# datemoon/ASR-decoder

Hardware: AMD Instinct MI355X
Metric: frames/sec decoded (RTFx = value/100) at fixed beam (higher is better)
Workload: dtype f32; 1 GPU; BASELINE configs[1]: batch=128 utterances/GPU x 300 frames, 10142717-arc HCLG, beam=13, max_active=1000000, min_active=0, 3000 pdfs; global_batch=128, frames_per_utt=300, parallelism=utterance-sharded x1 (graph replicated), channel_groups=3, degraded_frames=0, regime=beam-only pruning (max_active never binds, min_active 0): bi

## Files before the change

### asr-decoder_amd/csrc/wfst_kernels.hip

```cpp
#include <type_traits>

#include "wfst_device.h"

namespace wfst {

typedef unsigned long long u64;

__device__ __forceinline__ uint32_t f2o(float f) {
  uint32_t u = __float_as_uint(f);
  return u ^ ((u >> 31) ? 0xFFFFFFFFu : 0x80000000u);
}
__device__ __forceinline__ float o2f(uint32_t o) {
  uint32_t u = (o & 0x80000000u) ? (o ^ 0x80000000u) : ~o;
  return __uint_as_float(u);
}
template <class T>
__device__ __forceinline__ T ld_agent(const T *p) {
  return __hip_atomic_load(p, __ATOMIC_RELAXED, __HIP_MEMORY_SCOPE_AGENT);
}
__device__ __forceinline__ void lds_barrier() {
  asm volatile("s_waitcnt lgkmcnt(0)" ::: "memory");
  __builtin_amdgcn_s_barrier();
  asm volatile("" ::: "memory");
}
// ... 831 lines not shown
            const bool pseudo = pi >= 0;
            const int a = abeg_[q] + off;
            const int4 arc = arc_[q];
            const float base_cost = (cost_[q] + (-ll_[q])) + __int_as_float(arc.z);
            int4 rec;
            if (pseudo) {
              const int4 leaf = (j + 1 < S) ? s_arc[j + 1] : D.g.arcs[a + 1];
              float tt = base_cost;
              if (leaf.z == 1) {
                tt = tt + __int_as_float(leaf.y);
              } else if (leaf.z == 2) {
                tt = (tt + __int_as_float(leaf.w)) + __int_as_float(leaf.y);
              } else {
                const float *pw = D.g.pseudo_w + (size_t)arc.y * kPseudoDepthMax;
                for (int u = 0; u < leaf.z; ++u) tt = tt + pw[u];
              }
              rec = make_int4(arc.w, __float_as_int(tt), kPrevUnresolved, (int)((uint32_t)leaf.x | kEpsRec));
            } else {
              rec = make_int4(arc.w, __float_as_int(base_cost), tok0 + (super ? s_tidx[l] : l), (int)((uint32_t)a | flags_of((uint32_t)arc.y)));
              tmin = fminf(tmin, base_cost);
            }
            if (D.degcode) {
              const uint32_t code = (uint32_t)arc.x >> kColBits;
              rec.w = (int)(((uint32_t)rec.w & 0x3FFFFFFFu) | (code << 30));
              rec.z = pseudo ? kPrevUnresolved - (int)(code >> 2) : (int)((uint32_t)rec.z | ((code >> 2) << D.tok_idx_bits));
            }
            s_arc[j] = rec;
            cand_mask |= 1u << i;
            if (D.best_exp) {
              const u64 cb = ((u64)f2o(__int_as_float(rec.y)) << 32) | (uint32_t)rec.x;
              cbest = cb < cbest ? cb : cbest;
            }
          }
        }
        {
          const float wmin = wave_min_f(tmin);
          if (lane == 0 && wmin < kInf) atomicMin(&s_bound, f2o(wmin + ab));
          if (D.best_exp) {
            const u64 cv = cbest < best_seen ? cbest : ~0ull;
            if (__ballot(cv != ~0ull)) {
              const u64 wb = wave_min_u64(cv);
              if (lane == 0) atomicMin(&s_best, wb);
            }
          }
          lds_barrier();
          const uint32_t tb = s_bound;
          if (o2f(tb) < bound) {
            if (tid == 0) atomicMin(&ctl->bound, tb);
            bound = o2f(tb);
          }
          if (D.best_exp && tid == 0) {
            const u64 tbest = s_best;
            if (tbest < best_seen) atomicMin(&ctl->best_next, tbest);
          }
        }
        if constexpr (kTimers) { if (tid == 0) dbg_phase(D, 14, tq); }
        ST_FRESH_TID();
        int pr[kStIter];
#pragma unroll
        for (int i = 0; i < kStIter; ++i) {
          pr[i] = -1;
          if (!(cand_mask & (1u << i))) continue;
          const int j = (wave + i * (kStThreads / 64)) * 64 + lane;
          const int2 xy = *reinterpret_cast<const int2 *>(&s_arc[j]);
          if (__int_as_float(xy.y) < bound) {
            const int part = part_of(hash32(xy.x), log2part);
            pr[i] = (part << 16) | atomicAdd(&s_cnt[part], 1);
          }
        }
        lds_barrier();
        if (tid < 64) {
          const int cnt = tid < P ? s_cnt[tid] : 0;
          int g = 0;
          if (cnt) {
            g = atomicAdd(&bucket_cnt[tid], cnt);
            if (g + cnt > bcap) atomicOr(&ctl->error, kErrBucketFull);
          }
          s_gbase[tid] = g;
          s_cnt[tid] = 0;
          const uint32_t wrote = wave_sum_u32((uint32_t)cnt);
          if (tid == 0 && wrote) atomicAdd(&s_stat[2], wrote);
        }
        lds_barrier();
        if constexpr (kTimers) { if (tid == 0) dbg_phase(D, 15, tq); }
        ST_FRESH_TID();
#pragma unroll
        for (int i = 0; i < kStIter; ++i) {
          if (pr[i] < 0) continue;
          const int j = (wave + i * (kStThreads / 64)) * 64 + lane;
          const int p = pr[i] >> 16, gi = s_gbase[p] + (pr[i] & 0xFFFF);
          if (gi < bcap) bucket[(size_t)p * bcap + gi] = s_arc[j];
        }
        __syncthreads();
        if (tid == 0) { s_bound = 0xFFFFFFFFu; s_best = ~0ull; }
        if constexpr (kTimers) { if (tid == 0) dbg_phase(D, 16, tq); }
      }
      if ((rnd + 1) * kStTokens < n_live) {
        const bool exp = s_cost[tid] <= cutoff;
        const int nem = s_nemit[tid], zt = (s_base[tid + 1] - s_base[tid] - nem) >> 1;
        const uint32_t wN = (uint32_t)__popcll(__ballot(exp)), wE = wave_sum_u32(exp ? (uint32_t)nem : 0u),
                       wZ = wave_sum_u32(exp ? (uint32_t)zt : 0u);
        if (lane == 0) { if (wN) atomicAdd(&s_stat[0], wN); if (wE) atomicAdd(&s_stat[1], wE); if (wZ) atomicAdd(&s_stat[3], wZ); }
        __syncthreads();
      }
      }
    }
    {
      ST_FRESH_TID();
      const bool exp = counted && s_cost[tid] <= cutoff;
      const int nem = exp ? s_nemit[tid] : 0, zt = exp ? (s_base[tid + 1] - s_base[tid] - nem) >> 1 : 0;
      tile_tail(D, c, ctl, group, par, exp ? 1u : 0u, (uint32_t)nem, 0u, (uint32_t)zt, s_stat);
    }
    if (total_tiles <= (int)gridDim.x) break;
    if (tid == 0) s_ticket = (int)gridDim.x + atomicAdd(&fc->ticket[par], 1);
    __syncthreads();
    t = __builtin_amdgcn_readfirstlane(s_ticket);
    __syncthreads();
    if (t < total_tiles) td = tiles[t];
    if constexpr (kTimers) tq = wall_clock64();
  }
}
#undef ST_FRESH_TID
__global__ __launch_bounds__(kStThreads, 4) void expand_kernel_staged(DecoderDev D, int group, int par) { expand_staged_body<false, false>(D, group, par); }
__global__ __launch_bounds__(kStThreads, 4) void expand_kernel_staged_timed(DecoderDev D, int group, int par) { expand_staged_body<true, false>(D, group, par); }
#pragma clang diagnostic push
#pragma clang diagnostic ignored "-Wpass-failed"
__global__ __launch_bounds__(kStThreads, 5) void expand_kernel_staged_row(DecoderDev D, int group, int par) { expand_staged_body<false, true>(D, group, par); }
#pragma clang diagnostic pop
__global__ __launch_bounds__(kStThreads, 4) void expand_kernel_staged_row_timed(DecoderDev D, int group, int par) { expand_staged_body<true, true>(D, group, par); }

constexpr int kInsertThreads = 512;
#ifndef WFST_INSERT_UNROLL
#define WFST_INSERT_UNROLL 3
#endif
constexpr int kInsertUnroll = WFST_INSERT_UNROLL;
constexpr uint32_t kNoSlot = 0xFFFFu;
constexpr int kInsertPk = (kInsertUnroll + 1) / 2;
__device__ __forceinline__ void put16(uint32_t *p, int k, uint32_t v) {
  p[k >> 1] = (k & 1) ? (p[k >> 1] & 0xFFFFu) | (v << 16) : (p[k >> 1] & 0xFFFF0000u) | v;
}
__device__ __forceinline__ uint32_t get16(const uint32_t *p, int k) { return (k & 1) ? p[k >> 1] >> 16 : p[k >> 1] & 0xFFFFu; }

struct BoundaryLite {
  float redf[16];
  u64 best;
  int active, n, nd, front_begin, ntiles, tile_tokens, tile_start, pad_bits;
  uint32_t hist[256];
  uint32_t sel_prefix, sel_k;
  float prev_ab;
  u64 h_best;
  int h_risky;
  int h_nf, h_err;
  uint32_t h_bound;
};
template <int kT>
__device__ __forceinline__ void frame_boundary_fused(const DecoderDev &D, int c, const int32_t *target, int chan_cnt, int group,
                                                     int par_next, bool do_prep, BoundaryLite &sh, uint32_t *sel_cache, int sel_cache_cap);
template <int kT, bool kSc1, class Sh, int kKeep>
__device__ __forceinline__ float kth_smallest_t(const int4 *tok, int n, int k, Sh &sh, uint32_t *cache, int cache_cap, uint32_t lo_o, uint32_t hi_o);
#ifndef WFST_NOINLINE_COLD
#define WFST_COLD __forceinline__
#else
#define WFST_COLD __attribute__((noinline))
#endif
#ifndef WFST_COLD_KEEP
#define WFST_COLD_KEEP 4
#endif
template <int kT>
__device__ WFST_COLD float kth_smallest_cold(const int4 *tok, int n, int k, BoundaryLite *sh, uint32_t *cache, int cache_cap, uint32_t lo_o, uint32_t hi_o) {
  return kth_smallest_t<kT, true, BoundaryLite, WFST_COLD_KEEP>(tok, n, k, *sh, cache, cache_cap, lo_o, hi_o);
}

template <bool kLat, bool kBig, bool kFused>
__device__ __forceinline__ void insert_body(const DecoderDev &D, int group, int par, const int32_t *target = nullptr, int boundary = 0,
                                            int chan_cnt = 0) {
  constexpr bool kTwo = kFused && !kLat && !kBig;
  extern __shared__ __attribute__((aligned(16))) unsigned char smem[];
  const int tid = threadIdx.x, lane = tid & 63, wave = tid >> 6;
  const int SLmax = D.lds_slots;
  typedef typename std::conditional<kBig, u64, int32_t>::type KeyT;
  const KeyT kNoKey = (KeyT)~(KeyT)0;
  u64 *vals = reinterpret_cast<u64 *>(smem);
  KeyT *keys = reinterpret_cast<KeyT *>(smem + (size_t)SLmax * 8);
  int32_t *tidx = reinterpret_cast<int32_t *>(smem + (size_t)SLmax * (8 + sizeof(KeyT)));
  struct __attribute__((aligned(16))) InsertShared {
    int nstates, gpos, wpos, ok, item, pad[3];
    int lw[12];
    u64 best[kInsertThreads / 64];
    int pref[68];
  };
  static_assert(sizeof(InsertShared) % 16 == 0, "keep the dynamic LDS base aligned");
  __shared__ InsertShared ish;
  int &s_nstates = ish.nstates, &s_gpos = ish.gpos, &s_wpos = ish.wpos, &s_ok = ish.ok, &s_item = ish.item, &s_last = ish.pad[0];
  int &s_ech = ish.pad[1], &s_efill = ish.pad[2];
  constexpr bool kListEmit = kLat && kFused && !kBig;
  __shared__ BoundaryLite bsh;
  u64 *s_best = ish.best;
  int *s_pref = ish.pref;
  FrameCtl *fc = D.fctl + group;
  const int n_heavy = min(fc->n_items[par], D.item_cap / 2), n_items = n_heavy + min(fc->n_small[par], D.item_cap / 2);
  const int P = D.n_part;

  unsigned long long th = wall_clock64();
  for (int it = blockIdx.x; it < n_items;) {
  const int islot = __builtin_amdgcn_readfirstlane(it < n_heavy ? it : D.item_cap - 1 - (it - n_heavy));
  const int item = D.items[(size_t)group * D.item_cap + islot];
  const int my_pref = D.item_pref[((size_t)group * D.item_cap + islot) * 64 + lane];
  const int c = item >> 16, g0 = (item >> 8) & 0xFF, G = item & 0xFF;
  ChanCtl *ctl = D.ctl + c;
  int ech_reg = 0;
  if (kListEmit && tid == 0) {
    s_efill = 0;
    if (G) ech_reg = atomicAdd(&D.emit_cnt[c * 32], kEmitChunk);
  }
  int n = 0;
  {
    n = G ? __shfl(my_pref, G - 1, 64) : 0;
    if (wave == 0 && lane < G) s_pref[lane + 1] = my_pref;
    if (tid == 0) s_pref[0] = 0;
  }
  int log2g = 0;
  while ((1 << log2g) < G) ++log2g;
  const int log2grp = D.log2part - log2g;
  const int4 *bucket0 = D.bucket + ((size_t)c * P + g0) * D.bucket_cap;
  const int32_t *bucket_lm0 = kBig ? D.bucket_lm + ((size_t)c * P + g0) * D.bucket_cap : nullptr;
  const uint32_t bound_o = ctl->bound;
  const float cutoff = o2f(bound_o);
  const u64 best_early = (kTwo && D.best_exp) ? ctl->best_next : ~0ull;
  const int err_early = kTwo ? ctl->error : 0;
  const bool risky = kTwo && boundary && (ctl->items_left & kRiskyBit);
  int log2sl = 6;
  while ((1 << log2sl) < 4 * n && log2sl < D.log2lds) ++log2sl;
  const int SL = 1 << log2sl;
  const uint32_t mask = (uint32_t)SL - 1;
  const int base = ctl->front_begin + ctl->front_count;
  int4 *tok = D.tok + (size_t)c * D.arena_cap;
  u64 *evals = D.eps_vals + (size_t)c * D.ecap;
  int32_t *etoki = D.eps_toki + (size_t)c * D.ecap;
  int32_t *eocc = D.eps_occ_list + (size_t)c * D.wl_cap;
  int4 *wl = D.worklist + (size_t)c * 2 * D.wl_cap;
  u64 *occ_wl = reinterpret_cast<u64 *>(&ctl->eps_occ);

  int log2sub = 0;
  while (n > ((SL * 3) >> 2) << log2sub) ++log2sub;
  const int sub_shift = 32 - log2grp - log2sl - log2sub;
  if (sub_shift < 0 && tid == 0) atomicOr(&ctl->error, kErrTableFull);
  __syncthreads();
  auto load_rec = [&](int i, int *lm) -> int4 {
    *lm = 0;
    if (i >= n) return make_int4(0, 0x7F800000, 0, 0);
    int b = 0;
    if (G > 1) {
      int lo = 0, hi = G;
      while (hi - lo > 1) {
        const int mid = (lo + hi) >> 1;
        if (s_pref[mid] <= i) lo = mid; else hi = mid;
      }
      b = lo;
    }
    const size_t pos = (size_t)b * D.bucket_cap + (i - s_pref[b]);
    if constexpr (kBig) *lm = bucket_lm0[pos];
    return bucket0[pos];
  };
  auto key_of = [&](const int4 &r, int lm) -> KeyT {
    if constexpr (kBig) return big_key(r.x, lm);
    else return (KeyT)r.x;
  };
  auto hash_of = [&](const int4 &r, int lm) -> uint32_t { return kBig ? hash_big(r.x, lm) : hash32(r.x); };

  u64 best = ~0ull;
  if (tid == 0) dbg_phase(D, 22, th);
  unsigned long long tq = wall_clock64();
  for (int sub = 0; sub_shift >= 0 && sub < (1 << log2sub); ++sub) {
    __syncthreads();
    int4 r[kInsertUnroll];
    int rl[kInsertUnroll];
#pragma unroll
    for (int k = 0; k < kInsertUnroll; ++k) r[k] = load_rec(k * kInsertThreads + tid, &rl[k]);
    for (int i = tid; i < SL; i += kInsertThreads) { keys[i] = kNoKey; vals[i] = kEmptyVal; }
    if (tid == 0) { s_nstates = 0; s_wpos = 0; s_ok = 1; }
    __syncthreads();
    if (tid == 0) dbg_phase(D, 6, tq);
#ifndef WFST_RECORDS_AT_FIRST_USE
    if constexpr (kTwo) {
#pragma unroll
      for (int k = 0; k < kInsertUnroll; ++k) asm volatile("" ::"v"(r[k].x), "v"(r[k].y), "v"(r[k].z), "v"(r[k].w));
    }
#endif

    const bool one_sweep = n <= kInsertThreads * kInsertUnroll;
    const bool carry = one_sweep && SL <= 0x8000;
    uint32_t cs[kInsertPk];
#pragma unroll
    for (int j = 0; j < kInsertPk; ++j) cs[j] = ~0u;
    for (int i0 = 0; i0 < n; i0 += kInsertThreads * kInsertUnroll) {
      if (i0 > 0) {
#pragma unroll
        for (int k = 0; k < kInsertUnroll; ++k) r[k] = load_rec(i0 + k * kInsertThreads + tid, &rl[k]);
      }
#pragma unroll
      for (int k = 0; k < kInsertUnroll; ++k) {
        if (!(__int_as_float(r[k].y) < cutoff)) continue;
        const uint32_t h = hash_of(r[k], rl[k]);
        if (log2sub && (int)((h >> sub_shift) & ((1u << log2sub) - 1u)) != sub) continue;
        uint32_t slot = lds_slot_of(h, log2grp, log2sl);
        const KeyT key = key_of(r[k], rl[k]);
        bool found = false;
        for (int q = 0; q < SL; ++q) {
          KeyT kk = keys[slot];
          if (kk == kNoKey) {
            kk = atomicCAS(&keys[slot], kNoKey, key);
            if (kk == kNoKey) { atomicAdd(&s_nstates, 1); found = true; break; }
          }
          if (kk == key) { found = true; break; }
          slot = (slot + 1) & mask;
        }
        if (found) {
          atomicMin(&vals[slot], ((u64)f2o(__int_as_float(r[k].y)) << 32) | (uint32_t)r[k].w);
          put16(cs, k, slot & 0xFFFFu);
        } else atomicOr(&ctl->error, kErrTableFull);
      }
    }
    __syncthreads();
    if (tid == 0) dbg_phase(D, 7, tq);
    const int ns = s_nstates;
    if (tid == 0) {
      int g = atomicAdd(&ctl->new_count, ns);
      s_gpos = g;
      if constexpr (kListEmit) s_ech = ech_reg;
      if (!(kTwo && D.soft_limit) && g + ns > D.max_tok) { atomicOr(&ctl->error, kErrFrontierFull); s_ok = 0; }
      if ((int64_t)base + g + ns > D.arena_cap) { atomicOr(&ctl->error, kErrArenaFull); s_ok = 0; }
      if (kTwo && !s_ok) atomicOr(reinterpret_cast<u64 *>(&ctl->new_count), kFrameErrBit);
    }
    __syncthreads();
    if (!s_ok) break;
    if (tid == 0) dbg_phase(D, 8, tq);
    const int gpos = s_gpos;
    [[maybe_unused]] const __amdgpu_buffer_rsrc_t tok_rsrc = __builtin_amdgcn_make_buffer_rsrc((void *)(tok + base), 0, 0x7FFFFFF0, 0x00020000);

    auto slot_of = [&](int k) -> int {
      if (carry) {
        const uint32_t s = get16(cs, k);
        return s == kNoSlot ? -1 : (int)s;
      }
      if (!(__int_as_float(r[k].y) < cutoff)) return -1;
      const uint32_t h = hash_of(r[k], rl[k]);
      if (log2sub && (int)((h >> sub_shift) & ((1u << log2sub) - 1u)) != sub) return -1;
      uint32_t slot = lds_slot_of(h, log2grp, log2sl);
      const KeyT key = key_of(r[k], rl[k]);
      for (int q = 0; q < SL; ++q) {
        const KeyT kk = keys[slot];
        if (kk == key) return (int)slot;
        if (kk == kNoKey) break;
        slot = (slot + 1) & mask;
      }
      return -1;
    };

    bool big_win[kInsertUnroll];
#pragma unroll
    for (int k = 0; k < kInsertUnroll; ++k) big_win[k] = false;
    if constexpr (kBig) {
      if (one_sweep) {
        const u64 *pkeys = D.pair_keys + (size_t)c * D.pair_cap;
        const int32_t *src_lm = D.tok_lm + (size_t)c * D.arena_cap;
        const uint32_t idx_mask = D.tok_idx_bits >= 31 ? 0x7FFFFFFFu : ((1u << D.tok_idx_bits) - 1u);
        int bslot[kInsertUnroll];
        u64 bspk[kInsertUnroll];
#pragma unroll
        for (int k = 0; k < kInsertUnroll; ++k) {
          bslot[k] = -1; bspk[k] = 0ull;
          const int slot = slot_of(k);
          if (slot < 0) continue;
          const u64 packed = ((u64)f2o(__int_as_float(r[k].y)) << 32) | (uint32_t)r[k].w;
          if (vals[slot] == packed) {
            const uint32_t src = (uint32_t)r[k].z & idx_mask;
            const int32_t sp = src < (uint32_t)D.arena_cap ? src_lm[src] : -1;
            bslot[k] = slot;
            bspk[k] = (sp >= 0 && sp < D.pair_cap) ? ld_agent(&pkeys[sp]) : 0ull;
          }
        }
        __syncthreads();
#pragma unroll
        for (int k = 0; k < kInsertUnroll; ++k)
          if (bslot[k] >= 0) vals[bslot[k]] = kEmptyVal;
        __syncthreads();
#pragma unroll
        for (int k = 0; k < kInsertUnroll; ++k)
          if (bslot[k] >= 0) atomicMin(&vals[bslot[k]], bspk[k]);
        __syncthreads();
#pragma unroll
        for (int k = 0; k < kInsertUnroll; ++k)
          if (bslot[k] >= 0) big_win[k] = vals[bslot[k]] == bspk[k];
        __syncthreads();
#pragma unroll
        for (int k = 0; k < kInsertUnroll; ++k)
          if (big_win[k]) vals[bslot[k]] = ((u64)f2o(__int_as_float(r[k].y)) << 32) | (uint32_t)r[k].w;
        __syncthreads();
      }
    }

    for (int i0 = 0; i0 < n; i0 += kInsertThreads * kInsertUnroll) {
      if (!one_sweep) {
#pragma unroll
        for (int k = 0; k < kInsertUnroll; ++k) r[k] = load_rec(i0 + k * kInsertThreads + tid, &rl[k]);
#ifndef WFST_RECORDS_AT_FIRST_USE
        if constexpr (kTwo) {
#pragma unroll
          for (int k = 0; k < kInsertUnroll; ++k) asm volatile("" ::"v"(r[k].x), "v"(r[k].y), "v"(r[k].z), "v"(r[k].w));
        }
#endif
      }
      uint32_t wp[kInsertPk];
#pragma unroll
      for (int j = 0; j < kInsertPk; ++j) wp[j] = ~0u;
#pragma unroll
      for (int k = 0; k < kInsertUnroll; ++k) {
        bool winner = false;
        const int slot = slot_of(k);
        if (slot >= 0) {
          const u64 packed = ((u64)f2o(__int_as_float(r[k].y)) << 32) | (uint32_t)r[k].w;
          winner = vals[slot] == packed && (!(kBig && one_sweep) || big_win[k]) &&
                   (!(kFused || kBig) || atomicCAS(&vals[slot], packed, packed | 0xFFFFFFFFull) == packed);
        }
        const u64 wm = __ballot(winner);
        if (!wm) continue;
        int wb = 0;
        if (lane == 0) wb = atomicAdd(&s_wpos, __popcll(wm));
        wb = __builtin_amdgcn_readfirstlane(wb);
        if (winner) {
          put16(wp, k, (uint32_t)(wb + lane_rank(wm)));
          if (kLat) tidx[slot] = wb + lane_rank(wm);
        }
      }
#pragma unroll
      for (int k = 0; k < kInsertUnroll; ++k) {
        const uint32_t pos = get16(wp, k);
        const bool winner = pos != kNoSlot;
        const u64 wm = __ballot(winner);
        if (!wm) continue;
        const u64 packed = ((u64)f2o(__int_as_float(r[k].y)) << 32) | (uint32_t)r[k].w;
        int idx = 0;
        const uint32_t flags = (uint32_t)r[k].w & kFlagMask;
        if (winner) {
          idx = base + gpos + (int)pos;
          if (kTwo && risky) {
            typedef int v4i_t __attribute__((ext_vector_type(4)));
            const v4i_t v = {r[k].x, r[k].y, r[k].z, r[k].w};
            __builtin_amdgcn_raw_buffer_store_b128(v, tok_rsrc, (gpos + (int)pos) * 16, 0, 16);
          } else {
            tok[idx] = r[k];
          }
          if constexpr (kBig) D.tok_lm[(size_t)c * D.arena_cap + idx] = rl[k];
          if (!(kTwo && D.best_exp)) {
            const u64 b = (packed & 0xFFFFFFFF00000000ull) | (uint32_t)(kTwo ? r[k].x : idx);
            best = b < best ? b : best;
          }
        }
        if constexpr (kFused) {
          if constexpr (kLat) {
            if (winner && (flags & kFlagEpsTarget)) {
              const int ord = (int)((uint32_t)D.g.arcs[(uint32_t)r[k].w & kArcMask].y & 0x7FFFFFFFu) - 1;
              if (ord >= 0) etoki[ord] = idx;
            }
          }
          if constexpr (kListEmit) {
            const bool em = winner && (flags & kFlagOutEps);
            const u64 emm = __ballot(em);
            if (emm) {
              int eb = 0;
              if (lane == 0) eb = atomicAdd(&s_efill, __popcll(emm));
              eb = __shfl(eb, 0, 64);
              const int p = eb + lane_rank(emm);
// ... 712 lines not shown
      const u64 m = __ballot(incl > kk);
      const int owner = m ? __ffsll((long long)m) - 1 : 63;
      if (lane == owner) {
        uint32_t cum = incl - (c0 + c1 + c2 + c3);
        int b = 4 * lane;
        if (kk >= cum + c0) { cum += c0; ++b; if (kk >= cum + c1) { cum += c1; ++b; if (kk >= cum + c2) { cum += c2; ++b; } } }
        sh.sel_prefix = prefix | ((uint32_t)b << shift);
        sh.sel_k = kk - cum;
      }
    }
    __syncthreads();
  }
  return o2f(sh.sel_prefix);
}
__device__ __forceinline__ float kth_smallest(const int4 *tok, int n, int k, BoundaryShared &sh, uint32_t lo_o = 0u, uint32_t hi_o = 0xFFFFFFFFu) {
  return kth_smallest_t<kBT, false, BoundaryShared, kSelKeep>(tok, n, k, sh, nullptr, 0, lo_o, hi_o);
}

template <bool kBig>
__device__ __forceinline__ void prep_frame(const DecoderDev &D, int c, ChanCtl *ctl, const int32_t *target, BoundaryShared &sh,
                           int group, int par) {
  const int tid = threadIdx.x, lane = tid & 63, wave = tid >> 6;
  const float kInf = __builtin_huge_valf();
  unsigned long long tq = wall_clock64();
  if (tid == 0) {
    int act = (ctl->n_decoded < target[c]) && ctl->error == 0 && !ctl->finalized;
    if (act && ctl->n_decoded >= D.max_frames) { ctl->error |= kErrFramesFull; act = 0; }
    sh.active = act;
    if (!act) ctl->active = 0;
  }
  __syncthreads();
  if (!sh.active) return;
  const int n = ctl->front_count;
  const int4 *tokc = D.tok + (size_t)c * D.arena_cap;
  const int4 *tok = tokc + ctl->front_begin;
  const u64 best = ctl->best_next;
  const float best_w = n > 0 ? o2f((uint32_t)(best >> 32)) : kInf;

  float cutoff, ab;
  int super_k = 1;
  if (D.max_active == 2147483647 && D.min_active == 0 && !D.soft_limit) {
    ab = D.beam;
    cutoff = best_w + D.beam;
  } else {
    const float beam_cutoff = best_w + D.beam;
    float min_active_cutoff = kInf, max_active_cutoff = kInf;
    const uint32_t sel_lo = (D.fused && !kBig) ? f2o(best_w) : 0u, sel_hi = (D.fused && !kBig) ? ctl->bound : 0xFFFFFFFFu;
    const int max_eff = D.soft_limit ? min(D.max_active, D.max_tok) : D.max_active;
    if (n > max_eff) {
      max_active_cutoff = kth_smallest(tok, n, max_eff, sh, sel_lo, sel_hi);
      if (tid == 0 && D.soft_limit && D.max_tok < D.max_active) D.degraded[c] += 1;
      if (max_active_cutoff < beam_cutoff) super_k = super_tile_tokens(n, max_eff);
    }
    if (max_active_cutoff < beam_cutoff) {
      ab = max_active_cutoff - best_w + D.beam_delta;
      cutoff = max_active_cutoff;
    } else {
      if (n > D.min_active) {
        const bool below_beam = D.fused && !kBig && ctl->n_decoded > 0 && ctl->adaptive_beam == D.beam;
        if (D.min_active == 0 || below_beam) min_active_cutoff = best_w;
        else min_active_cutoff = kth_smallest(tok, n, D.min_active, sh, sel_lo, sel_hi);
      }
      if (min_active_cutoff > beam_cutoff) {
        ab = min_active_cutoff - best_w + D.beam_delta;
        cutoff = min_active_cutoff;
      } else {
        ab = D.beam;
        cutoff = beam_cutoff;
      }
    }
  }

  float seed = kInf;
  if (n > 0 && !(!kBig && D.seed_tiles)) {
    int4 bt;
    if (D.best_row) bt = make_int4((int)(uint32_t)best, __float_as_int(best_w), 0, 0);
    else bt = tokc[(uint32_t)best];
    const uint2 si = make_uint2((uint32_t)bt.x + 1u, (uint32_t)D.g.arcs[bt.x].x);
    const int deg = (int)(si.y >> kEpsBits), ab0 = (int)(si.x + (si.y & kEpsMask));
    const float *llrow = D.ll_base[c] + (size_t)ctl->n_decoded * D.stride;
    const float bc = __int_as_float(bt.y);
    const int blm = kBig ? D.tok_lm[(size_t)c * D.arena_cap + (uint32_t)best] : 0;
    for (int e = tid; e < deg; e += kBT) {
      const int4 arc = D.g.arcs[ab0 + e];
      float tot_score;
      if constexpr (kBig) {
        const int ol = D.g.arc_olabel[ab0 + e];
        int n1, n2;
        const float lm_score = ol != 0 ? lm_step(D, c, blm, ol, &n1, &n2) : 0.0f;
        tot_score = ((lm_score + bc) + __int_as_float(arc.z)) - llrow[arc.x & D.g.col_mask];
      } else {
        tot_score = (bc + __int_as_float(arc.z)) - llrow[arc.x & D.g.col_mask];
      }
      seed = fminf(seed, tot_score);
    }
  }
  seed = wave_min_f(seed);
  if (lane == 0) sh.redf[wave] = seed;
  __syncthreads();
  if (tid == 0) {
    float s = sh.redf[0];
    for (int w = 1; w < kBW; ++w) s = fminf(s, sh.redf[w]);
    const float next_cutoff = s + ab;
    ctl->cur_cutoff = cutoff;
    ctl->adaptive_beam = ab;
    ctl->bound = f2o(s < kInf ? next_cutoff : kInf);
    ctl->new_count = 0;
    ctl->best_next = ~0ull;
    ctl->active = 1;
    int tile_tokens = D.staged ? D.st_tile_tokens : kTileTokens;
    if ((int64_t)n * (int)gridDim.x <= 700ll * 256) tile_tokens = 256;
    if ((int64_t)n * (int)gridDim.x <= 700ll * 128) tile_tokens = 128;
    if (D.staged) tile_tokens = min(tile_tokens, D.st_tile_tokens);
    if (D.staged && !kBig && super_k > 1) tile_tokens = super_k;
    sh.tile_tokens = tile_tokens;
    const int ntiles = (n + tile_tokens - 1) / tile_tokens;
    sh.active = 0;
    const int nseed = (!kBig && D.seed_tiles && ntiles > 0) ? 1 : 0;
    ctl->tiles_left = ntiles + nseed;
    if (ntiles == 0 && D.two_launch) {
      ctl->items_left = ctl->stores_left = 1;
      push_empty_item(D, c, group, par);
    }
    if (ntiles > 0) {
      const int start = atomicAdd(&D.fctl[group].total_tiles[par], ntiles + nseed);
      if (start + ntiles + nseed <= D.tile_cap) { sh.sel_k = (uint32_t)start; sh.active = ntiles + nseed; }
      else ctl->error |= kErrFrontierFull;
    }
  }
  __syncthreads();
  const int ntl = sh.active;
  const int nseed = (!kBig && D.seed_tiles && ntl > 0) ? 1 : 0;
  TileDesc *tiles = D.tiles + (size_t)group * D.tile_cap + sh.sel_k;
  for (int i = tid; i < ntl; i += kBT) {
    TileDesc td;
    td.chan = c;
    const int k = i - nseed;
    td.tok_begin = ctl->front_begin + k * sh.tile_tokens;
    td.tok_count = min(sh.tile_tokens, n - k * sh.tile_tokens);
    td.cutoff = cutoff;
    td.adaptive_beam = ab;
    td.pad = (int32_t)ctl->bound;
    td.llrow = D.ll_base[c] + (size_t)ctl->n_decoded * D.stride;
    if (k < 0) {
      td.tok_begin = (int32_t)(uint32_t)best;
      td.tok_count = 0;
      td.cutoff = best_w;
    }
    tiles[i] = td;
  }
  if (tid == 0) dbg_phase(D, 5, tq);
}

template <int kT>
__device__ __forceinline__ void frame_boundary_fused(const DecoderDev &D, int c, const int32_t *target, int chan_cnt, int group,
                                                     int par_next, bool do_prep, BoundaryLite &sh, uint32_t *sel_cache, int sel_cache_cap) {
  int tid = threadIdx.x;
  asm volatile("" : "+v"(tid));
  const int lane = tid & 63, wave = tid >> 6;
  ChanCtl *ctl = D.ctl + c;
  const float kInf = __builtin_huge_valf();
  for (int i = tid; i < D.n_part; i += kT) D.bucket_cnt[(size_t)c * D.n_part + i] = 0;
  if (tid == 0) {
    const int f = ctl->n_decoded;
    const int base = ctl->front_begin + ctl->front_count;
    const uint32_t bound_o = sh.h_bound;
    int nf = sh.h_nf;
    const int err = sh.h_err;
    const u64 best = D.best_exp ? sh.h_best : ld_agent(&ctl->best_next);
    int add_err = 0;
    if ((!D.soft_limit && nf > D.max_tok) || (int64_t)base + nf > D.arena_cap) nf = 0;
    if (err) nf = 0;
    if (f + 2 > D.max_frames + 1) add_err = kErrFramesFull;
    else {
      D.frame_off[(size_t)c * (D.max_frames + 2) + f + 2] = base + nf;
      D.cutoff_hist[(size_t)c * (D.max_frames + 2) + f + 1] = o2f(bound_o);
    }
    ctl->cnt_tok += (u64)nf;
    if (nf > ctl->peak_tokens) ctl->peak_tokens = nf;
    sh.prev_ab = ctl->adaptive_beam;
    ctl->front_begin = base;
    ctl->front_count = nf;
    ctl->n_decoded = f + 1;
    ctl->active = 0;
    if (add_err) atomicOr(&ctl->error, add_err);
    int act = do_prep && (f + 1 < target[c]) && !(err | add_err) && !ctl->finalized;
    if (act && f + 1 >= D.max_frames) { atomicOr(&ctl->error, kErrFramesFull); act = 0; }
    sh.active = act;
    sh.n = nf;
    sh.nd = f + 1;
    sh.front_begin = base;
    sh.best = best;
  }
  __syncthreads();
  if (!sh.active) return;
  const int n = sh.n, nd = sh.nd;
  const u64 best = sh.best;
  const float best_w = n > 0 ? o2f((uint32_t)(best >> 32)) : kInf;
  const float beam_cutoff = best_w + D.beam;
  const int max_eff = D.soft_limit ? min(D.max_active, D.max_tok) : D.max_active;
#ifdef WFST_LEAN_BOUNDARY
  const bool need_max = false, need_min = false;
#else
  const bool need_max = n > max_eff;
  const bool need_min = D.min_active > 0 && n > D.min_active && !(sh.prev_ab == D.beam);
#endif
  float ab = D.beam, cutoff = beam_cutoff;
  if (need_max || need_min) {
    if (tid == 0) {
      if (!sh.h_risky) atomicOr(&ctl->error, kErrInternal);
      int spins = 0;
      while (sh.h_risky && ld_agent(&ctl->stores_left) != 0) {
        __builtin_amdgcn_s_sleep(4);
        if (++spins > (1 << 22)) { atomicOr(&ctl->error, kErrInternal); break; }
      }
      if (need_max && D.max_tok < D.max_active) D.degraded[c] += 1;
    }
    __syncthreads();
    const int4 *tok = D.tok + (size_t)c * D.arena_cap + sh.front_begin;
    float min_active_cutoff = kInf, max_active_cutoff = kInf;
    if (n > D.min_active) min_active_cutoff = best_w;
#pragma nounroll
    for (int stage = need_max ? 0 : 1; stage < 2; ++stage) {
      if (stage == 1 && !need_min) break;
      const float v = kth_smallest_cold<kT>(tok, n, stage == 0 ? max_eff : D.min_active, &sh, sel_cache, sel_cache_cap,
                                            f2o(best_w), sh.h_bound);
      if (stage == 0) {
        max_active_cutoff = v;
        if (max_active_cutoff < beam_cutoff) break;
      } else {
        min_active_cutoff = v;
      }
    }
    if (max_active_cutoff < beam_cutoff) {
      ab = max_active_cutoff - best_w + D.beam_delta;
      cutoff = max_active_cutoff;
    } else if (min_active_cutoff > beam_cutoff) {
      ab = min_active_cutoff - best_w + D.beam_delta;
      cutoff = min_active_cutoff;
    }
  } else if (n <= D.min_active) {
    if (kInf > beam_cutoff) { ab = kInf - best_w + D.beam_delta; cutoff = kInf; }
  }
  const float *llrow = D.ll_base[c] + (size_t)nd * D.stride;
  float seed = kInf;
  if (n > 0 && !D.seed_tiles) {
    const int brow = (int)(uint32_t)best;
    const uint32_t hx = (uint32_t)D.g.arcs[brow].x;
    const int deg = (int)(hx >> kEpsBits), ab0 = brow + 1 + (int)(hx & kEpsMask);
    for (int e = tid; e < deg; e += kT) {
      const int4 arc = D.g.arcs[ab0 + e];
      seed = fminf(seed, (best_w + __int_as_float(arc.z)) - llrow[arc.x & D.g.col_mask]);
    }
  }
  if (!D.seed_tiles) {
    seed = wave_min_f(seed);
    if (lane == 0) sh.redf[wave] = seed;
    __syncthreads();
  }
  if (tid == 0) {
    float s = kInf;
    if (!D.seed_tiles) for (int w = 0; w < kT / 64; ++w) s = fminf(s, sh.redf[w]);
    const float next_cutoff = s + ab;
    ctl->cur_cutoff = cutoff;
    ctl->adaptive_beam = ab;
    ctl->bound = f2o(s < kInf ? next_cutoff : kInf);
    ctl->new_count = 0;
    ctl->best_next = ~0ull;
    ctl->active = 1;
    int tile_tokens = D.staged ? D.st_tile_tokens : kTileTokens;
    if ((int64_t)n * chan_cnt <= 700ll * 256) tile_tokens = 256;
    if ((int64_t)n * chan_cnt <= 700ll * 128) tile_tokens = 128;
    if (D.staged) tile_tokens = min(tile_tokens, D.st_tile_tokens);
    if (D.staged && need_max && cutoff < beam_cutoff) tile_tokens = super_tile_tokens(n, max_eff);
    const int ntiles = (n + tile_tokens - 1) / tile_tokens;
    const int nseed = (D.seed_tiles && ntiles > 0) ? 1 : 0;
    sh.tile_tokens = tile_tokens;
    sh.ntiles = 0;
    ctl->tiles_left = ntiles + nseed;
    if (ntiles == 0) {
      ctl->items_left = ctl->stores_left = 1;
      push_empty_item(D, c, group, par_next);
    } else {
      const int start = atomicAdd(&D.fctl[group].total_tiles[par_next], ntiles + nseed);
      if (start + ntiles + nseed <= D.tile_cap) { sh.tile_start = start; sh.ntiles = ntiles + nseed; }
      else atomicOr(&ctl->error, kErrFrontierFull);
    }
    sh.pad_bits = (int32_t)f2o(s < kInf ? next_cutoff : kInf);
  }
  __syncthreads();
  const int ntl = sh.ntiles;
  TileDesc *tiles = D.tiles + (size_t)group * D.tile_cap + sh.tile_start;
  const int32_t pad_bits = sh.pad_bits;
  const int nseed = (D.seed_tiles && ntl > 0) ? 1 : 0;
  for (int i = tid; i < ntl; i += kT) {
    TileDesc td;
    td.chan = c;
    const int k = i - nseed;
    td.tok_begin = sh.front_begin + k * sh.tile_tokens;
    td.tok_count = min(sh.tile_tokens, n - k * sh.tile_tokens);
    td.cutoff = cutoff;
    td.adaptive_beam = ab;
    td.pad = pad_bits;
    td.llrow = llrow;
    if (k < 0) {
      td.tok_begin = (int32_t)(uint32_t)best;
      td.tok_count = 0;
      td.cutoff = best_w;
    }
    tiles[i] = td;
  }
}

constexpr int kPrLds = 16384;
#ifndef WFST_PR_CHUNK
#define WFST_PR_CHUNK 8192
#endif
constexpr int kPrChunk = WFST_PR_CHUNK;
#ifndef WFST_PR_SLABS
#define WFST_PR_SLABS 8
#endif
constexpr int kPrSlabs = WFST_PR_SLABS;
constexpr int kPrSlabBase = 40;
constexpr int kPrParInts = kPruneParInts;
constexpr int kPrRawCount = 32;
constexpr int kPrRawChg = 34;
#ifndef WFST_PR_RAW_J
#define WFST_PR_RAW_J 16
#endif
constexpr int kPrRawJ = WFST_PR_RAW_J;
constexpr int kClSlabWordAt = kClSlabWord;
constexpr int kPrRawPoison = 0x40000000;
static_assert(kPrRawChg + 3 <= kPrRawAbandon && kPrRawAbandonCount < kPrSlabBase, "prune_par: raw-pass words overlap");
static_assert(kPrSlabBase + 2 * kPrSlabs <= kClSlabWordAt, "prune_par: slab counts run into the closure launch's meeting word (WFST_PR_SLABS too large)");
static_assert(16 + 10 <= kPrRawCount, "prune_par: lattice_emit's counters [16, 26)");
static_assert(kClSlabWordAt % 2 == 0 && kClSlabWordAt + 2 <= kPruneParInts, "prune_par: the closure launch's 64-bit meeting word");
struct ScanShared {
  u64 red[2][kBT / 64];
  int changed, any_changed, cnt, err;
  int wsum[kBT / 64];
  int flag[3];
};
struct PruneShared : ScanShared {
  union {
    struct { uint2 e[kPrLds]; } w;
    int pre[kPrChunk + 1];
  };
};

__device__ __forceinline__ int block_exscan(int v, ScanShared &ps, int *total) {
  const int tid = threadIdx.x, lane = tid & 63, wave = tid >> 6;
  int incl = wave_incl_scan(v);
  __syncthreads();
  if (lane == 63) ps.wsum[wave] = incl;
  __syncthreads();
  int base = 0, tot = 0;
#pragma unroll
  for (int w = 0; w < kBT / 64; ++w) {
    const int x = ps.wsum[w];
    if (w < wave) base += x;
    tot += x;
  }
  *total = tot;
  return base + incl - v;
}

__device__ __forceinline__ float link_extra_of(int32_t link_delta, uint32_t eo, uint32_t cost_bits, int32_t w) {
  if (eo >= f2o(__builtin_huge_valf())) return __builtin_huge_valf();
  return o2f(eo) + (link_delta ? __int_as_float(w) : __int_as_float(w) - __uint_as_float(cost_bits));
}

template <bool kFinal, bool kSnap = false>
__device__ __forceinline__ void prune_pass(const DecoderDev &D, int c, PruneShared &ps, bool raw_done = false, int snap_use_final = 1) {
  static_assert(kFinal || !kSnap, "a snapshot is a FinalizeDecoding walk");
  const int tid = threadIdx.x, lane = tid & 63, wave = tid >> 6;
  ChanCtl *ctl = D.ctl + c;
  const int nd = ctl->n_decoded;
  int4 *tok = D.tok + (size_t)c * D.arena_cap;
  int4 *links = D.links + (size_t)c * D.link_cap;
  uint2 *extra = (kSnap ? D.snap_extra : D.extra) + (size_t)c * D.arena_cap;
  int32_t *remap = D.remap + (size_t)c * D.arena_cap;
  int32_t *foff = D.frame_off + (size_t)c * (D.max_frames + 2);
  int32_t *loff = D.link_off + (size_t)c * (D.max_frames + 3);
  int32_t *lmid = D.link_mid + (size_t)c * (D.max_frames + 3);
  const float kInf = __builtin_huge_valf();
  const uint32_t kInfO = f2o(kInf);
  const float lb = D.lattice_beam;
  if (ctl->error) return;
  unsigned long long tq = wall_clock64();
  const int n_prev = ctl->pruned_upto;
  const int fn = foff[nd], fn1 = foff[nd + 1];
  bool any_final = false;

  constexpr int kPU = 6;
  auto for_links = [&](int lo, int hi, auto &&f) {
    for (int i0 = lo; i0 < hi; i0 += kBT * kPU) {
      int4 L[kPU];
      u64 e[kPU];
#pragma unroll
      for (int u = 0; u < kPU; ++u) {
        const int i = i0 + u * kBT + tid;
        L[u] = i < hi ? links[i] : make_int4(-1, 0, 0, 0);
      }
#pragma unroll
      for (int u = 0; u < kPU; ++u) e[u] = L[u].x >= 0 ? ld_agent(reinterpret_cast<const u64 *>(&extra[L[u].y])) : 0ull;
#pragma unroll
      for (int u = 0; u < kPU; ++u) {
        if (L[u].x < 0) continue;
        const uint32_t eo = (uint32_t)e[u];
        const float le = link_extra_of(D.link_delta, eo, (uint32_t)(e[u] >> 32), L[u].w);
        f(i0 + u * kBT + tid, L[u], le);
      }
    }
  };
  auto relax_eps = [&](int e0, int e1) {
    if (e0 >= e1) return;
    for (int round = 0; round < 4096; ++round) {
      if (tid == 0) ps.changed = 0;
      __syncthreads();
      for_links(e0, e1, [&](int, const int4 &L, float le) {
        if (!(le <= lb)) return;
        if (le < 0.0f) le = 0.0f;
        const uint32_t o = f2o(le);
        if (o < atomicMin(&extra[L.x].x, o)) ps.changed = 1;
      });
      __syncthreads();
      const int ch = ps.changed;
      __syncthreads();
      if (!ch) break;
    }
    for_links(e0, e1, [&](int i, const int4 &, float le) {
      if (!kSnap && !(le <= lb)) links[i].x = -1;
    });
    __syncthreads();
  };

  if (kFinal) {
// ... 2205 lines not shown
```

Measured before the change: 2.385 million frames/s.

## Lockstep wave-wide hash probing and early tile reservation at frame boundary

Replaces the per-record sequential linear-probe loop in the fused insert path with a lockstep loop. It issues all unrolled CAS probes together, then counts newly claimed slots with a ballot instead of one LDS atomic per insert. It also caches per-channel control fields (target, finalized, n_decoded, base, adaptive beam) in LDS during insert, so the boundary does not reload them from global memory. The next-frame tile-range atomicAdd is issued speculatively at the start of the boundary to hide its latency. The cost is extra dummy CAS traffic for lanes with nothing pending and more complex control logic. Correctness depends on the early-reservation predicate matching the later one.

Measured after the change: 2.405 million frames/s (median of 4 runs). Within noise of the previous version (+0.8%).

```diff
diff --git a/asr-decoder_amd/csrc/wfst_kernels.hip b/asr-decoder_amd/csrc/wfst_kernels.hip
--- a/asr-decoder_amd/csrc/wfst_kernels.hip
+++ b/asr-decoder_amd/csrc/wfst_kernels.hip
@@ -1007,7 +1007,11 @@
   int h_risky;
   int h_nf, h_err;
   uint32_t h_bound;
+  int h_target, h_final, h_nd, h_base;
+  float h_prev_ab;
+  int h_pad[3];
 };
+static_assert(sizeof(BoundaryLite) % 16 == 0, "keep the dynamic LDS base aligned");
 template <int kT>
 __device__ __forceinline__ void frame_boundary_fused(const DecoderDev &D, int c, const int32_t *target, int chan_cnt, int group,
                                                      int par_next, bool do_prep, BoundaryLite &sh, uint32_t *sel_cache, int sel_cache_cap);
@@ -1030,6 +1034,7 @@
 __device__ __forceinline__ void insert_body(const DecoderDev &D, int group, int par, const int32_t *target = nullptr, int boundary = 0,
                                             int chan_cnt = 0) {
   constexpr bool kTwo = kFused && !kLat && !kBig;
+  constexpr bool kLockstep = kTwo;
   extern __shared__ __attribute__((aligned(16))) unsigned char smem[];
   const int tid = threadIdx.x, lane = tid & 63, wave = tid >> 6;
   const int SLmax = D.lds_slots;
@@ -1084,6 +1089,9 @@
   const u64 best_early = (kTwo && D.best_exp) ? ctl->best_next : ~0ull;
   const int err_early = kTwo ? ctl->error : 0;
   const bool risky = kTwo && boundary && (ctl->items_left & kRiskyBit);
+  int e_target = 0, e_final = 0, e_nd = 0;
+  float e_ab = 0.0f;
+  if (kTwo && boundary) { e_target = target[c]; e_final = ctl->finalized; e_nd = ctl->n_decoded; e_ab = ctl->adaptive_beam; }
   int log2sl = 6;
   while ((1 << log2sl) < 4 * n && log2sl < D.log2lds) ++log2sl;
   const int SL = 1 << log2sl;
@@ -1101,6 +1109,9 @@
   const int sub_shift = 32 - log2grp - log2sl - log2sub;
   if (sub_shift < 0 && tid == 0) atomicOr(&ctl->error, kErrTableFull);
   __syncthreads();
+  if (kTwo && boundary && tid == 0) {
+    bsh.h_target = e_target; bsh.h_final = e_final; bsh.h_nd = e_nd; bsh.h_base = base; bsh.h_prev_ab = e_ab;
+  }
   auto load_rec = [&](int i, int *lm) -> int4 {
     *lm = 0;
     if (i >= n) return make_int4(0, 0x7F800000, 0, 0);
@@ -1153,6 +1164,46 @@
 #pragma unroll
         for (int k = 0; k < kInsertUnroll; ++k) r[k] = load_rec(i0 + k * kInsertThreads + tid, &rl[k]);
       }
+      if constexpr (kLockstep) {
+        uint32_t ps[kInsertUnroll];
+        uint32_t pend = 0, claimed = 0;
+#pragma unroll
+        for (int k = 0; k < kInsertUnroll; ++k) {
+          ps[k] = (uint32_t)(tid + k * kInsertThreads) & mask;
+          if (!(__int_as_float(r[k].y) < cutoff)) continue;
+          const uint32_t h = hash_of(r[k], rl[k]);
+          if (log2sub && (int)((h >> sub_shift) & ((1u << log2sub) - 1u)) != sub) continue;
+          ps[k] = lds_slot_of(h, log2grp, log2sl);
+          pend |= 1u << k;
+        }
+        for (int q = 0; __any(pend != 0) && q < SL; ++q) {
+          KeyT kk[kInsertUnroll];
+#pragma unroll
+          for (int k = 0; k < kInsertUnroll; ++k) {
+            const KeyT key = key_of(r[k], rl[k]);
+            kk[k] = atomicCAS(&keys[ps[k]], ((pend >> k) & 1u) ? kNoKey : key, key);
+          }
+#pragma unroll
+          for (int k = 0; k < kInsertUnroll; ++k) asm volatile("" : "+v"(kk[k]));
+#pragma unroll
+          for (int k = 0; k < kInsertUnroll; ++k) {
+            if (!((pend >> k) & 1u)) continue;
+            if (kk[k] == kNoKey) claimed |= 1u << k;
+            if (kk[k] == kNoKey || kk[k] == key_of(r[k], rl[k])) {
+              atomicMin(&vals[ps[k]], ((u64)f2o(__int_as_float(r[k].y)) << 32) | (uint32_t)r[k].w);
+              put16(cs, k, ps[k] & 0xFFFFu);
+              pend &= ~(1u << k);
+            } else {
+              ps[k] = (ps[k] + 1) & mask;
+            }
+          }
+        }
+        if (pend) atomicOr(&ctl->error, kErrTableFull);
+        int nw = 0;
+#pragma unroll
+        for (int k = 0; k < kInsertUnroll; ++k) nw += __popcll(__ballot((claimed >> k) & 1u));
+        if (lane == 0 && nw) atomicAdd(&s_nstates, nw);
+      } else {
 #pragma unroll
       for (int k = 0; k < kInsertUnroll; ++k) {
         if (!(__int_as_float(r[k].y) < cutoff)) continue;
@@ -1174,6 +1225,7 @@
           atomicMin(&vals[slot], ((u64)f2o(__int_as_float(r[k].y)) << 32) | (uint32_t)r[k].w);
           put16(cs, k, slot & 0xFFFFu);
         } else atomicOr(&ctl->error, kErrTableFull);
+      }
       }
     }
     __syncthreads();
@@ -2192,6 +2244,13 @@
   if (tid == 0) dbg_phase(D, 5, tq);
 }
 
+__device__ __forceinline__ int plain_tile_tokens(const DecoderDev &D, int n, int chan_cnt) {
+  int tile_tokens = D.staged ? D.st_tile_tokens : kTileTokens;
+  if ((int64_t)n * chan_cnt <= 700ll * 256) tile_tokens = 256;
+  if ((int64_t)n * chan_cnt <= 700ll * 128) tile_tokens = 128;
+  if (D.staged) tile_tokens = min(tile_tokens, D.st_tile_tokens);
+  return tile_tokens;
+}
 template <int kT>
 __device__ __forceinline__ void frame_boundary_fused(const DecoderDev &D, int c, const int32_t *target, int chan_cnt, int group,
                                                      int par_next, bool do_prep, BoundaryLite &sh, uint32_t *sel_cache, int sel_cache_cap) {
@@ -2200,10 +2259,31 @@
   const int lane = tid & 63, wave = tid >> 6;
   ChanCtl *ctl = D.ctl + c;
   const float kInf = __builtin_huge_valf();
+  int early = 0, early_start = 0, early_tt = 0, early_nt = 0;
+  if (tid == 0) {
+    const int f = sh.h_nd;
+    int nf = sh.h_nf;
+    if ((!D.soft_limit && nf > D.max_tok) || (int64_t)sh.h_base + nf > D.arena_cap || sh.h_err) nf = 0;
+    const bool act = do_prep && (f + 1 < sh.h_target) && !sh.h_err && !(f + 2 > D.max_frames + 1) && !sh.h_final && f + 1 < D.max_frames;
+    const int max_eff = D.soft_limit ? min(D.max_active, D.max_tok) : D.max_active;
+#ifdef WFST_LEAN_BOUNDARY
+    const bool limits = false;
+#else
+    const bool limits = nf > max_eff || (D.min_active > 0 && nf > D.min_active && !(sh.h_prev_ab == D.beam));
+#endif
+    if (act && !limits && nf > 0) {
+      const int tile_tokens = plain_tile_tokens(D, nf, chan_cnt);
+      const int ntiles = (nf + tile_tokens - 1) / tile_tokens;
+      int pn = par_next;
+      asm volatile("" : "+v"(pn));
+      early_start = atomicAdd(&D.fctl[group].total_tiles[pn], ntiles + (D.seed_tiles ? 1 : 0));
+      early = 1; early_tt = tile_tokens; early_nt = ntiles;
+    }
+  }
   for (int i = tid; i < D.n_part; i += kT) D.bucket_cnt[(size_t)c * D.n_part + i] = 0;
   if (tid == 0) {
-    const int f = ctl->n_decoded;
-    const int base = ctl->front_begin + ctl->front_count;
+    const int f = sh.h_nd;
+    const int base = sh.h_base;
     const uint32_t bound_o = sh.h_bound;
     int nf = sh.h_nf;
     const int err = sh.h_err;
@@ -2218,13 +2298,13 @@
     }
     ctl->cnt_tok += (u64)nf;
     if (nf > ctl->peak_tokens) ctl->peak_tokens = nf;
-    sh.prev_ab = ctl->adaptive_beam;
+    sh.prev_ab = sh.h_prev_ab;
     ctl->front_begin = base;
     ctl->front_count = nf;
     ctl->n_decoded = f + 1;
     ctl->active = 0;
     if (add_err) atomicOr(&ctl->error, add_err);
-    int act = do_prep && (f + 1 < target[c]) && !(err | add_err) && !ctl->finalized;
+    int act = do_prep && (f + 1 < sh.h_target) && !(err | add_err) && !sh.h_final;
     if (act && f + 1 >= D.max_frames) { atomicOr(&ctl->error, kErrFramesFull); act = 0; }
     sh.active = act;
     sh.n = nf;
@@ -2308,12 +2388,9 @@
     ctl->new_count = 0;
     ctl->best_next = ~0ull;
     ctl->active = 1;
-    int tile_tokens = D.staged ? D.st_tile_tokens : kTileTokens;
-    if ((int64_t)n * chan_cnt <= 700ll * 256) tile_tokens = 256;
-    if ((int64_t)n * chan_cnt <= 700ll * 128) tile_tokens = 128;
-    if (D.staged) tile_tokens = min(tile_tokens, D.st_tile_tokens);
+    int tile_tokens = early ? early_tt : plain_tile_tokens(D, n, chan_cnt);
     if (D.staged && need_max && cutoff < beam_cutoff) tile_tokens = super_tile_tokens(n, max_eff);
-    const int ntiles = (n + tile_tokens - 1) / tile_tokens;
+    const int ntiles = early ? early_nt : (n + tile_tokens - 1) / tile_tokens;
     const int nseed = (D.seed_tiles && ntiles > 0) ? 1 : 0;
     sh.tile_tokens = tile_tokens;
     sh.ntiles = 0;
@@ -2322,7 +2399,7 @@
       ctl->items_left = ctl->stores_left = 1;
       push_empty_item(D, c, group, par_next);
     } else {
-      const int start = atomicAdd(&D.fctl[group].total_tiles[par_next], ntiles + nseed);
+      const int start = early ? early_start : atomicAdd(&D.fctl[group].total_tiles[par_next], ntiles + nseed);
       if (start + ntiles + nseed <= D.tile_cap) { sh.tile_start = start; sh.ntiles = ntiles + nseed; }
       else atomicOr(&ctl->error, kErrFrontierFull);
     }
```
